# stateless-consensus/phant

Measured on AMD Instinct MI355X. Metric: mpt_proofs_verified_per_sec_depth8, higher is better.
Workload: dtype u64; 1 GPU; config3: 100000 synthetic depth-8 account proofs per GPU against one state root (7 x 532 B full branches + 112 B leaf, 3868 B and 29 Keccak-f per proof, 1% corrupted/exclusion, no cross-proof dedup); every launch sequence in flight verifies its own witness (seeds 2..3: distinct data per slot), 30 back-to-back passes per timed step; parallelism=key-sharded x1, verify_mode=flat, streams=2

## Files before the change

### phant_amd/csrc/mpt_verify_v3.hip

```cpp
#include <phant_platform.h>

#include "launch.h"
#include "mpt_verify_one.hip.h"
#include "coop_sponge.hip.h"
#include "verify_hash.hip.h"

namespace phant {
namespace v3 {
using namespace vh;

constexpr uint32_t HDR_PFN_BROKEN = 9;
constexpr uint32_t HDR_SLOW = 10;
constexpr uint32_t HDR_OPENED = 11;
constexpr uint32_t HDR_PARITY = 15;
constexpr uint32_t HDR_STAT = 1024;
constexpr uint32_t HDR_STAT_STRIPES = 16;
constexpr uint32_t HDR_STAT_WORDS = HDR_STAT_STRIPES * N_CLASS;
constexpr uint32_t HDR_STAT_END = HDR_STAT + 2u * HDR_STAT_WORDS;
constexpr uint32_t HDR_CUR = 256;
constexpr uint32_t HDR_WORDS = 768;
constexpr size_t HEADER_BYTES = 8192;
static_assert(HDR_STAT_END <= VERIFY_HEADER_WORDS && 4u * VERIFY_HEADER_WORDS <= HEADER_BYTES,
              "capi.hip copies VERIFY_HEADER_WORDS words back for the statistics");

PHANT_DEV uint32_t cursor_word(uint32_t cls, uint32_t stripe) { return HDR_CUR + 32u * stripe + cls; }



PHANT_DEV uint64_t key_prefix64(const uint8_t* __restrict__ key, uint32_t key_len) {
    uint64_t kb = 0;
    const uint32_t take = key_len < 8u ? key_len : 8u;
    for (uint32_t t = 0; t < take; ++t) kb |= (uint64_t)key[t] << (56u - 8u * t);
    return kb;
}
PHANT_DEV uint64_t key_prefix64_wide(const uint8_t* __restrict__ key, uint32_t key_len) {
    if (key_len < 8u) return key_prefix64(key, key_len);
    struct __attribute__((packed, aligned(1))) U64u { unsigned long long v; };
    return __builtin_bswap64(reinterpret_cast<const U64u*>(key)->v);
}
PHANT_DEV bool same_prefix(uint64_t x, uint64_t y, uint32_t d) { return d == 0u || ((x ^ y) >> (64u - 4u * d)) == 0ull; }
PHANT_DEV uint64_t group_hash(uint64_t kb, uint32_t root, uint32_t d) {
    const uint64_t pre = d ? (kb >> (64u - 4u * d)) : 0ull;
    uint64_t h = pre ^ ((uint64_t)(d + 1u) << 58) ^ ((uint64_t)root * 0x9E3779B97F4A7C15ull);
    h ^= h >> 33;
    h *= 0xff51afd7ed558ccdull;
    h ^= h >> 33;
    h *= 0xc4ceb9fe1a85ec53ull;
    h ^= h >> 33;
    return h;
}
PHANT_DEV uint32_t direct_index(uint64_t kb, uint32_t root, uint32_t d, uint32_t n_roots) {
    uint32_t width = 1u, below = 0u;
    for (uint32_t t = 0; t < d; ++t) {
        below += width;
        width <<= 4;
    }
    const uint32_t pre = d ? (uint32_t)(kb >> (64u - 4u * d)) : 0u;
    return n_roots * below + root * width + pre;
}
PHANT_DEV uint32_t slot_a(uint64_t h, uint32_t mask) { return (uint32_t)h & mask; }
PHANT_DEV uint32_t slot_b(uint64_t h, uint32_t mask) { return (uint32_t)(h >> 24) & mask; }

struct Args {
    VerifyArgs v;
    uint32_t total_nodes;
    uint32_t shallow;
    uint32_t direct;
    uint32_t* dtab;
    uint64_t* table;
    uint32_t tmask;
    uint32_t* rep;
    uint2* ent;
    uint32_t stripe_cap;
    uint32_t* hdr;
    uint32_t* digest;
    uint8_t* nstat;
};

PHANT_DEV void beside_the_hashing() { __builtin_amdgcn_s_setprio(3); }

__global__ void __launch_bounds__(256) zero_kernel(uint4* p, size_t n16, uint32_t* fail_count, uint32_t n_roots) {
    beside_the_hashing();
    const size_t i = (size_t)blockIdx.x * 256u + threadIdx.x;
    if (i < n16) p[i] = make_uint4(0u, 0u, 0u, 0u);
    if (fail_count)
        for (size_t r = i; r < n_roots; r += (size_t)gridDim.x * 256u) fail_count[r] = 0u;
}

struct ShallowLane {
    uint32_t p, d, j, root, len;
    uint64_t kb;
    bool act;
    bool valid;
    bool group;
    bool broken;
};
PHANT_DEV ShallowLane shallow_node(const Args& a, uint32_t p, uint32_t d) {
    ShallowLane L;
    L.p = p;
    L.d = d;
    L.j = 0;
    L.root = 0;
    L.len = 0;
    L.kb = 0;
    L.act = L.valid = L.group = L.broken = false;
    if (L.p >= a.v.n) return L;
    const uint32_t first = a.v.proof_first_node[L.p], last = a.v.proof_first_node[L.p + 1];
    if (last < first) {
        L.broken = L.d == 0u;
        return L;
    }
    if (last > a.total_nodes) return L;
    const uint32_t nn = 2u * a.v.key_len, cnt = last - first;
    const uint32_t end = cnt <= nn ? cnt : nn + 1u;
    if (L.d >= end) return L;
    L.act = true;
    L.j = first + L.d;
    L.root = a.v.root_idx ? a.v.root_idx[L.p] : 0u;
    const uint64_t e = a.v.node_off[L.j + 1], b = a.v.node_off[L.j];
    if (e >= b && e <= a.v.nodes_len && e - b <= 0x7fffffffull) {
        L.valid = true;
        L.len = (uint32_t)(e - b);
    }
    L.group = L.valid && L.len >= RATE && L.root < a.v.n_roots;
    if (L.group) L.kb = key_prefix64(a.v.keys + (uint64_t)a.v.key_len * L.p, a.v.key_len);
    return L;
}
PHANT_DEV ShallowLane shallow_lane(const Args& a, uint32_t g) {
    const uint32_t p = g / a.shallow;
    return shallow_node(a, p, g - p * a.shallow);
}

PHANT_DEV void clear_launch_state(const Args& a, uint32_t g, size_t lanes) {
    const uint32_t other = HDR_STAT + HDR_STAT_WORDS * ((a.hdr[HDR_PARITY] & 1u) ^ 1u);
    for (size_t i = g; i < HDR_WORDS + HDR_STAT_WORDS; i += lanes) {
        if (i < HDR_WORDS) {
            if (i != HDR_PARITY) a.hdr[i] = 0u;
        } else {
            a.hdr[other + (i - HDR_WORDS)] = 0u;
        }
    }
    if (a.v.fail_count)
        for (size_t r = g; r < a.v.n_roots; r += lanes) a.v.fail_count[r] = 0u;
}

__global__ void __launch_bounds__(256) propose_kernel(const Args a) {
    beside_the_hashing();
    const uint32_t g = blockIdx.x * 256u + threadIdx.x;
    clear_launch_state(a, g, (size_t)gridDim.x * 256u);
    const ShallowLane L = shallow_lane(a, g);
    if (L.act) a.nstat[L.j] = 0u;
    if (!L.group) return;
    if (L.d < a.direct) {
        a.dtab[direct_index(L.kb, L.root, L.d, a.v.n_roots)] = L.j + 1u;
    } else {
        const uint64_t h = group_hash(L.kb, L.root, L.d);
        const uint64_t entry = ((uint64_t)L.p << 32) | (uint64_t)(L.j + 1u);
        a.table[slot_a(h, a.tmask)] = entry;
        a.table[slot_b(h, a.tmask)] = entry;
    }
}

PHANT_DEV bool entry_matches(const Args& a, uint64_t en, const ShallowLane& L, uint32_t& node) {
    const uint32_t pr = (uint32_t)(en >> 32), j1 = (uint32_t)en;
    if (j1 == 0u || pr >= a.v.n) return false;
    node = j1 - 1u;
    if (pr == L.p) return node == L.j;
    const uint32_t f = a.v.proof_first_node[pr], l = a.v.proof_first_node[pr + 1];
    if (l < f || l > a.total_nodes || node < f || node >= l || node - f != L.d) return false;
    if ((a.v.root_idx ? a.v.root_idx[pr] : 0u) != L.root) return false;
    return same_prefix(key_prefix64(a.v.keys + (uint64_t)a.v.key_len * pr, a.v.key_len), L.kb, L.d);
}

PHANT_DEV uint64_t ent_index(const Args& a, uint32_t cls, uint32_t stripe, uint32_t at) {
    return ((uint64_t)cls * STRIPES + stripe) * a.stripe_cap + at;
}

PHANT_DEV bool wave_bytes_equal(const uint8_t* x, const uint8_t* y, uint32_t len, uint32_t lane) {
    uint32_t diff = 0;
    const uint32_t full = len & ~15u;
    for (uint32_t o = 16u * lane; o < full; o += 1024u) {
        const uint4 p = load16u(x + o), q = load16u(y + o);
        diff |= (p.x ^ q.x) | (p.y ^ q.y) | (p.z ^ q.z) | (p.w ^ q.w);
    }
    if (lane < (len & 15u)) diff |= (uint32_t)(x[full + lane] ^ y[full + lane]);
    return __ballot(diff != 0) == 0ull;
}

constexpr int COMPARE_UNROLL = 4;

__global__ void __launch_bounds__(256) PHANT_NUM_VGPR(48) dedup_kernel(const Args a) {
    constexpr uint32_t WAVES = 4;
    __shared__ uint32_t s_cnt[WAVES][N_LIST];
    __shared__ uint32_t s_base[N_LIST];
    beside_the_hashing();
    const uint32_t tid = threadIdx.x, lane = tid & 63u, wave = tid >> 6;
    const uint32_t NT = a.total_nodes;
    if (tid < WAVES * N_LIST) (&s_cnt[0][0])[tid] = 0u;
    const ShallowLane L = shallow_lane(a, blockIdx.x * 256u + tid);
    if (L.broken) a.hdr[HDR_PFN_BROKEN] = 1u;

    const uint32_t j = L.j;
    uint32_t cand = j;
    uint64_t b = 0, cb = 0;
    if (L.group) {
        uint32_t c = j;
        if (L.d < a.direct) {
            const uint32_t t = a.dtab[direct_index(L.kb, L.root, L.d, a.v.n_roots)];
            if (t) c = t - 1u;
        } else {
            const uint64_t h = group_hash(L.kb, L.root, L.d);
            uint32_t node;
            if (entry_matches(a, a.table[slot_a(h, a.tmask)], L, node)) c = node;
            else if (entry_matches(a, a.table[slot_b(h, a.tmask)], L, node)) c = node;
        }
        if (c != j && c < NT) {
            const uint64_t c0 = a.v.node_off[c], c1 = a.v.node_off[c + 1];
            if (c1 >= c0 && c1 <= a.v.nodes_len && c1 - c0 == L.len) {
                cand = c;
                cb = c0;
                b = a.v.node_off[j];
            }
        }
    }

    const uint32_t coff = 16u * (lane & 31u);
    const bool upper = lane >= 32u;
    const uint32_t b_lo = (uint32_t)b, b_hi = (uint32_t)(b >> 32), cb_lo = (uint32_t)cb, cb_hi = (uint32_t)(cb >> 32);
    bool differs = false;
    const bool is532 = cand != j && L.len == BRANCH_LEN;
    unsigned long long todo = __ballot(is532);
    while (todo) {
        uint32_t i0[COMPARE_UNROLL], i1[COMPARE_UNROLL];
        uint4 x[COMPARE_UNROLL], y[COMPARE_UNROLL];
        uint32_t i = 0;
#pragma unroll
        for (int u = 0; u < COMPARE_UNROLL; ++u) {
            if (todo) {
                i = (uint32_t)__builtin_ctzll(todo);
                todo &= todo - 1ull;
            }
            i0[u] = i;
            if (todo) {
                i = (uint32_t)__builtin_ctzll(todo);
                todo &= todo - 1ull;
            }
            i1[u] = i;
            const uint64_t own0 = lane_u64(b_lo, b_hi, i0[u]), own1 = lane_u64(b_lo, b_hi, i1[u]);
            const uint64_t oth0 = lane_u64(cb_lo, cb_hi, i0[u]), oth1 = lane_u64(cb_lo, cb_hi, i1[u]);
            x[u] = load16u(a.v.nodes + (upper ? own1 : own0) + coff);
            y[u] = load16u(a.v.nodes + (upper ? oth1 : oth0) + coff);
        }
#pragma unroll
        for (int u = 0; u < COMPARE_UNROLL; ++u) {
            uint32_t diff = x[u].x ^ y[u].x;
            diff = __builtin_amdgcn_bitop3_b32(x[u].y, y[u].y, diff, 0xBE);
            diff = __builtin_amdgcn_bitop3_b32(x[u].z, y[u].z, diff, 0xBE);
            diff = __builtin_amdgcn_bitop3_b32(x[u].w, y[u].w, diff, 0xBE);
            const unsigned long long m = __ballot(diff != 0);
            if ((uint32_t)m != 0u && lane == i0[u]) differs = true;
            if ((uint32_t)(m >> 32) != 0u && lane == i1[u]) differs = true;
        }
    }
    if (is532 && !differs) {
        const uint8_t* const own = a.v.nodes + b + (BRANCH_LEN - 28u);
        const uint8_t* const oth = a.v.nodes + cb + (BRANCH_LEN - 28u);
        const uint4 p0 = load16u(own), p1 = load16u(own + 12), q0 = load16u(oth), q1 = load16u(oth + 12);
        uint32_t diff = (p0.x ^ q0.x) | (p0.y ^ q0.y) | (p0.z ^ q0.z) | (p0.w ^ q0.w);
        diff |= (p1.x ^ q1.x) | (p1.y ^ q1.y) | (p1.z ^ q1.z) | (p1.w ^ q1.w);
        if (diff) differs = true;
    }
    todo = __ballot(cand != j && L.len != BRANCH_LEN);
    while (todo) {
        const uint32_t i = (uint32_t)__builtin_ctzll(todo);
        todo &= todo - 1ull;
        const uint32_t ll = lane_u32(L.len, i);
        const bool eq = wave_bytes_equal(a.v.nodes + lane_u64(b_lo, b_hi, i), a.v.nodes + lane_u64(cb_lo, cb_hi, i), ll, lane);
        if (lane == i && !eq) differs = true;
    }
    if (differs) cand = j;
    if (L.act) a.rep[j] = cand;

    const uint32_t cls = (L.act && L.valid && cand == j) ? node_list(L.len) : CLASS_NONE;
    uint32_t my_rank = 0;
    __syncthreads();
    todo = __ballot(cls != CLASS_NONE);
    while (todo) {
        const uint32_t c0 = lane_u32(cls, (uint32_t)__builtin_ctzll(todo));
        const unsigned long long m = __ballot(cls == c0);
        if (lane == 0) s_cnt[wave][c0] = (uint32_t)__popcll(m);
        if (cls == c0) my_rank = (uint32_t)__popcll(m & ((1ull << lane) - 1ull));
        todo &= ~m;
    }
    __syncthreads();
    const uint32_t stripe = blockIdx.x % STRIPES;
    if (tid < N_LIST) {
        uint32_t tot = 0;
        for (uint32_t w = 0; w < WAVES; ++w) tot += s_cnt[w][tid];
        s_base[tid] = tot ? atomicAdd(&a.hdr[cursor_word(tid, stripe)], tot) : 0u;
    }
    __syncthreads();
    if (cls != CLASS_NONE) {
        uint32_t at = s_base[cls] + my_rank;
        for (uint32_t w = 0; w < wave; ++w) at += s_cnt[w][cls];
        a.ent[ent_index(a, cls, stripe, at)] = make_uint2(j, L.p);
    }
}


PHANT_DEV const uint8_t* ref_location(const Args& a, uint32_t j, uint32_t d, uint32_t root, uint32_t nib_parent, uint64_t b) {
    if (d == 0u) return root < a.v.n_roots ? a.v.roots + 32ull * root : nullptr;
    if (nib_parent >= 16u) return nullptr;
    const uint64_t pb = a.v.node_off[j - 1u];
    if (pb > b || b - pb != BRANCH_LEN) return nullptr;
    return a.v.nodes + pb + (4u + 33u * nib_parent);
}

struct RefBytes { uint4 lo, hi; };
PHANT_DEV RefBytes load_ref(const uint8_t* q) {
    RefBytes r;
    r.lo = r.hi = make_uint4(0, 0, 0, 0);
    if (q) {
        r.lo = load16u(q);
        r.hi = load16u(q + 16);
    }
    return r;
}
PHANT_DEV bool digest_equals(const Sponge& s, const RefBytes& r) {
    const uint32_t diff = (s.lo[0] ^ r.lo.x) | (s.hi[0] ^ r.lo.y) | (s.lo[1] ^ r.lo.z) | (s.hi[1] ^ r.lo.w) |
                          (s.lo[2] ^ r.hi.x) | (s.hi[2] ^ r.hi.y) | (s.lo[3] ^ r.hi.z) | (s.hi[3] ^ r.hi.w);
    return diff == 0u;
}
PHANT_DEV void store_node_digest(const Args& a, uint32_t j, const Sponge& s) {
    uint4* o = reinterpret_cast<uint4*>(a.digest + 8ull * j);
    o[0] = make_uint4(s.lo[0], s.hi[0], s.lo[1], s.hi[1]);
    o[1] = make_uint4(s.lo[2], s.hi[2], s.lo[3], s.hi[3]);
}


PHANT_DEV bool list_role(const Args& a, uint32_t q, const uint32_t lane) {
    static_assert(N_QUEUE > 64u && N_QUEUE <= 128u, "two lists per lane");
    const uint32_t cnt_a = a.hdr[cursor_word(queue_class(lane), lane % STRIPES)];
    const uint32_t cnt_b = lane + 64u < N_QUEUE ? a.hdr[cursor_word(queue_class(lane + 64u), (lane + 64u) % STRIPES)] : 0u;
    const uint32_t ch_a = (cnt_a + 63u) / 64u, ch_b = (cnt_b + 63u) / 64u;
    const uint32_t incl_a = wave_inclusive_scan(ch_a, lane);
    uint32_t li, before, cnt;
    const unsigned long long m_a = __ballot(q < incl_a);
    if (m_a) {
        const uint32_t l = (uint32_t)__builtin_ctzll(m_a);
        li = l;
        before = lane_u32(incl_a, l) - lane_u32(ch_a, l);
        cnt = lane_u32(cnt_a, l);
    } else {
        const uint32_t incl_b = lane_u32(incl_a, 63u) + wave_inclusive_scan(ch_b, lane);
        const unsigned long long m_b = __ballot(q < incl_b);
        if (!m_b) return false;
        const uint32_t l = (uint32_t)__builtin_ctzll(m_b);
        li = l + 64u;
        before = lane_u32(incl_b, l) - lane_u32(ch_b, l);
        cnt = lane_u32(cnt_b, l);
    }
    const uint32_t cls = queue_class(li), stripe = li % STRIPES;
    uint32_t idx = (q - before) * 64u + lane;
    idx = idx < cnt ? idx : cnt - 1u;
    const uint2 en = a.ent[ent_index(a, cls, stripe, idx)];
    const uint32_t j = en.x;
    const uint8_t* const safe_end = a.v.nodes + a.v.nodes_len;
    const uint64_t b = a.v.node_off[j];
    const uint32_t len = (uint32_t)(a.v.node_off[j + 1] - b);
    const uint8_t* const p = a.v.nodes + b;

    const uint8_t* refp = nullptr;
    {
        const uint32_t owner = en.y;
        const uint32_t d = j - a.v.proof_first_node[owner];
        const uint32_t root = a.v.root_idx ? a.v.root_idx[owner] : 0u;
        uint32_t nibp = 16u;
        if (d >= 1u && d - 1u < 2u * a.v.key_len) nibp = key_nibble(a.v.keys + (uint64_t)a.v.key_len * owner, d - 1u);
        refp = ref_location(a, j, d, root, nibp, b);
    }
    const RefBytes ref = load_ref(refp);

    Sponge s;
    uint32_t bad;
    const uint32_t len0 = (uint32_t)__builtin_amdgcn_readfirstlane(len);
    if (cls == LIST_B532) {
        bad = hash_b532<true>(s, p);
    } else if (cls == 0u && __ballot(len != len0 || p + RATE > safe_end) == 0ull) {
        hash_short_uniform(s, p, len0);
        bad = 1u;
    } else {
        hash_any(s, p, len, safe_end);
        bad = 1u;
    }
    uint32_t ns = NS_HASHED | (bad == 0u ? NS_CANON : 0u);
    if (refp) ns |= NS_LINK_CHECKED | (digest_equals(s, ref) ? NS_LINK_OK : 0u);
    a.nstat[j] = (uint8_t)ns;
    store_node_digest(a, j, s);
    return true;
}

constexpr uint32_t DEEP_LEVELS = 8;

template <bool SOLO>
PHANT_DEV void deep_role(const Args& a, const uint32_t w, const uint32_t lane, const uint32_t waves_per_level, const uint32_t levels,
                         uint32_t (&s_ref)[8][256]) {
    const uint32_t level = w / waves_per_level;
    if (level >= levels) return;
    const uint32_t p = (w % waves_per_level) * 64u + lane;
    const uint8_t* const safe_end = a.v.nodes + a.v.nodes_len;
    const uint32_t nn = 2u * a.v.key_len;
    uint32_t hashed[N_CLASS] = {0, 0, 0, 0, 0, 0, 0, 0};
    const uint32_t stat_buf = a.hdr[HDR_PARITY] & 1u;
    for (uint32_t d = a.shallow + level;; d += levels) {
        uint32_t first = 0, count = 0, root = 0;
        if (p < a.v.n) {
            first = a.v.proof_first_node[p];
            const uint32_t last = a.v.proof_first_node[p + 1];
            if (last >= first && last <= a.total_nodes) count = last - first;
            if constexpr (SOLO) {
                if (last < first) a.hdr[HDR_PFN_BROKEN] = 1u;
            }
            if (a.v.root_idx) root = a.v.root_idx[p];
        }
        if (__ballot(d < count) == 0ull) break;
        const uint32_t j = first + d;
        bool active = d < count;
        uint64_t b = 0;
        uint32_t len = 0;
        if (active) {
            const uint64_t e = a.v.node_off[j + 1];
            b = a.v.node_off[j];
            active = e >= b && e <= a.v.nodes_len && e - b <= 0x7fffffffull;
            len = active ? (uint32_t)(e - b) : 0u;
            if (!active) a.nstat[j] = 0u;
        }
        const bool roomy = a.v.nodes_len >= BRANCH_LEN;
        const uint8_t* const ptr = a.v.nodes + (active ? b : 0ull);
        const uint8_t* refp = nullptr;
        if (active) {
            const uint8_t* const key = a.v.keys + (uint64_t)a.v.key_len * p;
            const uint32_t nibp = (d >= 1u && d - 1u < nn) ? key_nibble(key, d - 1u) : 16u;
            refp = ref_location(a, j, d, root, nibp, b);
        }
        {
            const RefBytes ref = load_ref(refp);
            const uint32_t t = threadIdx.x;
            s_ref[0][t] = ref.lo.x; s_ref[1][t] = ref.lo.y; s_ref[2][t] = ref.lo.z; s_ref[3][t] = ref.lo.w;
            s_ref[4][t] = ref.hi.x; s_ref[5][t] = ref.hi.y; s_ref[6][t] = ref.hi.z; s_ref[7][t] = ref.hi.w;
        }
        {
            const uint32_t cls = len / RATE < N_CLASS ? len / RATE : N_CLASS - 1u;
#pragma unroll
            for (uint32_t c = 0; c < N_CLASS; ++c) hashed[c] += (uint32_t)__popcll(__ballot(active && cls == c));
        }
        enum : uint32_t { F_ACTIVE = 1u, F_REF = 2u, F_CANON = 4u };
        uint32_t flags = (active ? F_ACTIVE : 0u) | (refp != nullptr ? F_REF : 0u);
        Sponge s;
        const bool is532 = active && len == BRANCH_LEN;
        if (roomy && __ballot(is532) != 0ull) {
            const uint32_t bad = hash_b532<true>(s, is532 ? ptr : a.v.nodes);
            if (is532 && bad == 0u) flags |= F_CANON;
        }
        const bool rest = active && !(roomy && is532);
        if (__ballot(rest) != 0ull) {
            const uint32_t len0 = (uint32_t)__builtin_amdgcn_readfirstlane(len);
            if (len0 < RATE && __ballot(!rest || len != len0 || ptr + RATE > safe_end) == 0ull) {
                hash_short_uniform(s, ptr, len0);
            } else if (rest) {
                hash_any(s, ptr, len, safe_end);
            }
        }
        if (flags & F_ACTIVE) {
            const uint32_t j = a.v.proof_first_node[p] + d;
            uint32_t ns = NS_HASHED | ((flags & F_CANON) ? NS_CANON : 0u);
            if (flags & F_REF) {
                const uint32_t t = threadIdx.x;
                RefBytes ref;
                ref.lo = make_uint4(s_ref[0][t], s_ref[1][t], s_ref[2][t], s_ref[3][t]);
                ref.hi = make_uint4(s_ref[4][t], s_ref[5][t], s_ref[6][t], s_ref[7][t]);
                ns |= NS_LINK_CHECKED | (digest_equals(s, ref) ? NS_LINK_OK : 0u);
            }
            a.nstat[j] = (uint8_t)ns;
            store_node_digest(a, j, s);
        }
    }
    if (lane < N_CLASS) {
        uint32_t mine = 0;
#pragma unroll
        for (uint32_t c = 0; c < N_CLASS; ++c) mine = lane == c ? hashed[c] : mine;
        if (mine) atomicAdd(&a.hdr[HDR_STAT + HDR_STAT_WORDS * stat_buf + N_CLASS * (w % HDR_STAT_STRIPES) + lane], mine);
    }
}

template <bool SOLO>
__global__ void __launch_bounds__(256, 4) hash_deep_kernel(const Args a, const uint32_t waves_per_level, const uint32_t levels) {
    __shared__ uint32_t s_ref[8][256];
    const uint32_t w = (uint32_t)__builtin_amdgcn_readfirstlane(blockIdx.x * 4u + (threadIdx.x >> 6));
    deep_role<SOLO>(a, w, threadIdx.x & 63u, waves_per_level, levels, s_ref);
}
constexpr uint32_t COOP_MAX_NODES = 2048;
constexpr uint32_t WAVE_MAX_NODES = 2048;
constexpr uint32_t NO_STAT = 0xffffffffu;
PHANT_DEV void coop_node(const Args& a, const CoopLane& c, const uint32_t l, const uint32_t base, const bool present, const uint32_t p,
                         const uint32_t j, const uint32_t d, const uint32_t root, const uint32_t stat_word) {
    struct __attribute__((packed, aligned(1))) U64 { unsigned long long v; };
    const uint32_t nn = 2u * a.v.key_len;
    bool active = false;
    uint32_t len = 0;
    uint64_t b = 0;
    if (present) {
        const uint64_t e = a.v.node_off[j + 1];
        b = a.v.node_off[j];
        active = e >= b && e <= a.v.nodes_len && e - b <= 0x7fffffffull;
        len = active ? (uint32_t)(e - b) : 0u;
        if (!active && l == 0) a.nstat[j] = 0u;
    }
    const uint8_t* const ptr = a.v.nodes + (active ? b : 0ull);
    const uint8_t* refp = nullptr;
    if (active) {
        const uint8_t* const key = a.v.keys + (uint64_t)a.v.key_len * p;
        refp = ref_location(a, j, d, root, (d >= 1u && d - 1u < nn) ? key_nibble(key, d - 1u) : 16u, b);
    }
    const uint32_t nb = active ? len / RATE + 1u : 0u;
    const uint32_t nb_other = __shfl(nb, (int)(base ^ 32u), 64);
    const uint32_t nb_max = nb > nb_other ? nb : nb_other;
    const bool branch = active && len == BRANCH_LEN;
    uint32_t lo = 0, hi = 0, dlo = 0, dhi = 0, bad = 0;
    for (uint32_t k = 0; k < nb_max; ++k) {
        if (k < nb && l < 17u) {
            const uint32_t off = k * RATE + 8u * l;
            unsigned long long w = 0;
            if (off + 8u <= len) {
                w = reinterpret_cast<const U64*>(ptr + off)->v;
            } else {
#pragma unroll
                for (uint32_t t = 0; t < 8u; ++t) {
                    const uint32_t q = off + t;
                    if (q < len) w |= (unsigned long long)ptr[q] << (8u * t);
                    else if (q == len) w |= 0x01ull << (8u * t);
                }
            }
            if (k + 1u == nb && l == 16u) w |= 0x80ull << 56;
            if (branch) {
#pragma unroll
                for (uint32_t t = 0; t < 8u; ++t) {
                    const uint32_t q = off + t;
                    const uint32_t byte = (uint32_t)(w >> (8u * t)) & 0xffu;
                    const int want = q == 0u ? 0xf9 : q == 1u ? 0x02 : q == 2u ? 0x11 : q == BRANCH_LEN - 1u ? 0x80 : (q < BRANCH_LEN && (q - 3u) % 33u == 0u) ? 0xa0 : -1;
                    if (want >= 0 && byte != (uint32_t)want) bad = 1u;
                }
            }
            lo ^= (uint32_t)w;
            hi ^= (uint32_t)(w >> 32);
        }
        coop_permute(c, lo, hi);
        if (k + 1u == nb) {
            dlo = lo;
            dhi = hi;
        }
    }
    bool ne = false;
    if (refp && l < 4u) {
        const unsigned long long r = reinterpret_cast<const U64*>(refp + 8u * l)->v;
        ne = (uint32_t)r != dlo || (uint32_t)(r >> 32) != dhi;
    }
    const uint32_t any_bad = (uint32_t)(__ballot(bad != 0u) >> base), any_ne = (uint32_t)(__ballot(ne) >> base);
    if (active) {
        uint32_t ns = NS_HASHED | ((branch && any_bad == 0u) ? NS_CANON : 0u);
        if (refp) ns |= NS_LINK_CHECKED | (any_ne == 0u ? NS_LINK_OK : 0u);
        if (l < 4u) {
            a.digest[8ull * j + 2u * l] = dlo;
            a.digest[8ull * j + 2u * l + 1u] = dhi;
        }
        if (l == 0) {
            a.nstat[j] = (uint8_t)ns;
            const uint32_t cls = len / RATE < N_CLASS ? len / RATE : N_CLASS - 1u;
            if (stat_word != NO_STAT) atomicAdd(&a.hdr[stat_word + cls], 1u);
        }
    }
}

__global__ void __launch_bounds__(256) hash_coop_kernel(const Args a, const uint32_t levels) {
    const uint32_t tid = threadIdx.x, l = tid & 31u, base = tid & 32u;
    const uint32_t h = blockIdx.x * (blockDim.x >> 5) + (tid >> 5);
    const uint32_t p = h / levels, level = h % levels;
    uint32_t first = 0, count = 0, root = 0;
    if (p < a.v.n) {
        first = a.v.proof_first_node[p];
        const uint32_t last = a.v.proof_first_node[p + 1];
        if (last >= first && last <= a.total_nodes) count = last - first;
        if (last < first && l == 0) a.hdr[HDR_PFN_BROKEN] = 1u;
        if (a.v.root_idx) root = a.v.root_idx[p];
    }
    const uint32_t stat_word = HDR_STAT + HDR_STAT_WORDS * (a.hdr[HDR_PARITY] & 1u) + N_CLASS * (h % HDR_STAT_STRIPES);
    const CoopLane c = coop_lane(l, base, gridDim.x * (blockDim.x >> 6) <= 1024u);
    for (uint32_t d = level;; d += levels) {
        if (__ballot(d < count) == 0ull) break;
        coop_node(a, c, l, base, d < count, p, first + d, d, root, stat_word);
    }
}

PHANT_DEV void wave_node(const Args& a, const WaveLane& c, const uint32_t l, const uint32_t p, const uint32_t j, const uint32_t d, const uint32_t root,
                         const uint32_t stat_word) {
    struct __attribute__((packed, aligned(1))) U64 { unsigned long long v; };
    const uint32_t nn = 2u * a.v.key_len;
    const uint64_t e = a.v.node_off[j + 1], b = a.v.node_off[j];
    const bool active = e >= b && e <= a.v.nodes_len && e - b <= 0x7fffffffull;
    if (!active) {
        if (l == 0) a.nstat[j] = 0u;
        return;
    }
    const uint32_t len = (uint32_t)(e - b);
    const uint8_t* const ptr = a.v.nodes + b;
    const uint8_t* const key = a.v.keys + (uint64_t)a.v.key_len * p;
    const uint8_t* const refp = ref_location(a, j, d, root, (d >= 1u && d - 1u < nn) ? key_nibble(key, d - 1u) : 16u, b);
    const uint32_t nb = len / RATE + 1u;
    const bool branch = len == BRANCH_LEN;
    uint32_t lo = 0, hi = 0, bad = 0;
    for (uint32_t k = 0; k < nb; ++k) {
        if (c.word < 17u) {
            const uint32_t off = k * RATE + 8u * c.word;
            unsigned long long w = 0;
            if (off + 8u <= len) {
                w = reinterpret_cast<const U64*>(ptr + off)->v;
            } else {
#pragma unroll
                for (uint32_t t = 0; t < 8u; ++t) {
                    const uint32_t q = off + t;
                    if (q < len) w |= (unsigned long long)ptr[q] << (8u * t);
                    else if (q == len) w |= 0x01ull << (8u * t);
                }
            }
            if (k + 1u == nb && c.word == 16u) w |= 0x80ull << 56;
            if (branch) {
#pragma unroll
                for (uint32_t t = 0; t < 8u; ++t) {
                    const uint32_t q = off + t;
                    const uint32_t byte = (uint32_t)(w >> (8u * t)) & 0xffu;
                    const int want = q == 0u ? 0xf9 : q == 1u ? 0x02 : q == 2u ? 0x11 : q == BRANCH_LEN - 1u ? 0x80 : (q < BRANCH_LEN && (q - 3u) % 33u == 0u) ? 0xa0 : -1;
                    if (want >= 0 && byte != (uint32_t)want) bad = 1u;
                }
            }
            lo ^= (uint32_t)w;
            hi ^= (uint32_t)(w >> 32);
        }
        wave_permute(c, lo, hi);
    }
    bool ne = false;
    if (refp && l < 4u) {
        const unsigned long long r = reinterpret_cast<const U64*>(refp + 8u * l)->v;
        ne = (uint32_t)r != lo || (uint32_t)(r >> 32) != hi;
    }
    const bool any_bad = __ballot(bad != 0u) != 0ull, any_ne = __ballot(ne) != 0ull;
    uint32_t ns = NS_HASHED | ((branch && !any_bad) ? NS_CANON : 0u);
    if (refp) ns |= NS_LINK_CHECKED | (!any_ne ? NS_LINK_OK : 0u);
    if (l < 4u) {
        a.digest[8ull * j + 2u * l] = lo;
        a.digest[8ull * j + 2u * l + 1u] = hi;
    }
    if (l == 0) {
        a.nstat[j] = (uint8_t)ns;
        const uint32_t cls = len / RATE < N_CLASS ? len / RATE : N_CLASS - 1u;
        if (stat_word != NO_STAT) atomicAdd(&a.hdr[stat_word + cls], 1u);
    }
}

__global__ void __launch_bounds__(256) hash_wave_kernel(const Args a, const uint32_t levels) {
    const uint32_t tid = threadIdx.x, l = tid & 63u;
    const uint32_t h = blockIdx.x * (blockDim.x >> 6) + (tid >> 6);
    const uint32_t p = h / levels, level = h % levels;
    if (p >= a.v.n) return;
    const uint32_t first = a.v.proof_first_node[p], last = a.v.proof_first_node[p + 1];
    uint32_t count = 0;
    if (last >= first && last <= a.total_nodes) count = last - first;
    if (last < first && l == 0) a.hdr[HDR_PFN_BROKEN] = 1u;
    const uint32_t root = a.v.root_idx ? a.v.root_idx[p] : 0u;
    const uint32_t stat_word = HDR_STAT + HDR_STAT_WORDS * (a.hdr[HDR_PARITY] & 1u) + N_CLASS * (h % HDR_STAT_STRIPES);
    const WaveLane c = wave_lane(l);
    for (uint32_t d = level; d < count; d += levels) wave_node(a, c, l, p, first + d, d, root, stat_word);
}

__global__ void __launch_bounds__(256, 4) hash_list_kernel(const Args a) {
    __builtin_amdgcn_s_setprio(2);
    const uint32_t q = (uint32_t)__builtin_amdgcn_readfirstlane(blockIdx.x * 4u + (threadIdx.x >> 6));
    (void)list_role(a, q, threadIdx.x & 63u);
}

enum : uint32_t { LINK_GENERIC = 0, LINK_FAST = 1, LINK_HASH_OK = 2, LINK_BAD_HASH = 3 };

PHANT_DEV uint32_t code_of(uint32_t ns, bool has_nibble) {
    if (!(ns & NS_HASHED) || !(ns & NS_LINK_CHECKED)) return LINK_GENERIC;
    if (!(ns & NS_LINK_OK)) return LINK_BAD_HASH;
    return (has_nibble && (ns & NS_CANON)) ? LINK_FAST : LINK_HASH_OK;
}


template <bool DIRECT>
__global__ void __launch_bounds__(256) walk_kernel(const Args a) {
    __shared__ uint32_t s_stage[256 * WALK_SLOT_DW];
    beside_the_hashing();
    const uint32_t i = blockIdx.x * 256u + threadIdx.x;
    const bool in = i < a.v.n;
    uint32_t status = PHANT_PROOF_PRESENT;
    uint32_t r = 0;
    if (in) {
        uint32_t* const slot = s_stage + threadIdx.x * WALK_SLOT_DW;
        const uint8_t* const slot_node = reinterpret_cast<const uint8_t*>(slot);
        const uint8_t* const nodes_end = a.v.nodes + a.v.nodes_len;
        uint64_t voff = 0;
        uint32_t vlen = 0;
        const uint32_t first = a.v.proof_first_node[i], last = a.v.proof_first_node[i + 1];
        r = a.v.root_idx ? a.v.root_idx[i] : 0u;
        if (last < first || last > a.total_nodes || r >= a.v.n_roots) {
            status = PHANT_PROOF_BAD_INPUT;
        } else if (last == first) {
            uint32_t rw[8];
            GlobalBytes rb{a.v.roots + 32ull * r};
#pragma unroll
            for (int k = 0; k < 8; ++k) rw[k] = rb.u32(4 * k);
            status = is_empty_root(rw) ? PHANT_PROOF_ABSENT : PHANT_PROOF_INVALID_EMPTY;
        } else if (a.hdr[HDR_PFN_BROKEN] != 0u) {
            status = STATUS_NEEDS_SLOW;
        } else {
            const uint8_t* const key = a.v.keys + (uint64_t)a.v.key_len * i;
            const uint32_t nn = 2u * a.v.key_len;
            uint32_t sx = 0;
            if constexpr (!DIRECT) {
                const uint32_t cnt = last - first, end = cnt <= nn ? cnt : nn + 1u;
                sx = end < a.shallow ? end : a.shallow;
            }
            const uint8_t* const slot_key = reinterpret_cast<const uint8_t*>(slot + WALK_STAGE_BYTES / 4);
            const bool key_in_lds = a.v.key_len <= WALK_KEY_BYTES;
            if (key_in_lds) {
                uint8_t* kdst = reinterpret_cast<uint8_t*>(slot + WALK_STAGE_BYTES / 4);
                for (uint32_t t = 0; t < a.v.key_len; ++t) kdst[t] = key[t];
            }
            WalkState w;
            w.pos = 0;
            w.status = PHANT_PROOF_BAD_INPUT;
            w.value_pay = w.value_len = w.ref_pay = w.ref_total = 0;
            uint32_t used = first;
            status = 0xffffffffu;

            bool hash_known = false;
            uint32_t rprev = 0;
            for (bool run = true; run && used < last;) {
                const uint32_t base = used, dbase = used - first;
                const uint8_t* lp = a.nstat + base;
                const uint32_t c0 = load4u(lp), c1 = load4u(lp + 4);
                uint32_t rj[8], nsr[8], rpar[8];
                if constexpr (!DIRECT) {
                    if (dbase < sx) {
                        const uint8_t* rp = reinterpret_cast<const uint8_t*>(a.rep + base);
                        const uint4 r0 = load16u(rp), r1 = load16u(rp + 16);
                        rj[0] = r0.x; rj[1] = r0.y; rj[2] = r0.z; rj[3] = r0.w;
                        rj[4] = r1.x; rj[5] = r1.y; rj[6] = r1.z; rj[7] = r1.w;
#pragma unroll
                        for (int u = 0; u < 8; ++u) {
                            const bool sh = dbase + u < sx && base + u < last && rj[u] < a.total_nodes;
                            rj[u] = sh ? rj[u] : base + u;
                        }
#pragma unroll
                        for (int u = 0; u < 8; ++u) {
                            const bool copy = rj[u] != base + u;
                            nsr[u] = copy ? a.nstat[rj[u]] : 0u;
                            rpar[u] = (copy && rj[u] >= 1u && dbase + u >= 1u) ? a.rep[rj[u] - 1u] : 0xffffffffu;
                        }
                    } else {
#pragma unroll
                        for (int u = 0; u < 8; ++u) {
                            rj[u] = base + u;
                            nsr[u] = 0u;
                            rpar[u] = 0xffffffffu;
                        }
                    }
                }
#pragma unroll
                for (int u = 0; u < 8; ++u) {
                    if (!run || used >= last) continue;
                    const uint32_t own = ((u < 4 ? c0 : c1) >> (8 * (u & 3))) & 0xffu;
                    uint32_t c, me = used;
                    if constexpr (DIRECT) {
                        c = code_of(own, w.pos < nn);
                    } else {
                        me = rj[u];
                        if (me == used) c = code_of(own, w.pos < nn);
                        else if (used == first || rpar[u] == rprev) c = code_of(nsr[u], w.pos < nn);
                        else if (!(nsr[u] & NS_HASHED)) c = LINK_GENERIC;
                        else {
                            const uint8_t* rb = a.v.nodes + a.v.node_off[used - 1u] + (4u + 33u * key_nibble(key, w.pos - 1u));
                            const uint4 w0 = load16u(rb), w1 = load16u(rb + 16);
                            const uint4* dg = reinterpret_cast<const uint4*>(a.digest + 8ull * me);
                            const uint4 d0 = dg[0], d1 = dg[1];
                            const uint32_t diff = (d0.x ^ w0.x) | (d0.y ^ w0.y) | (d0.z ^ w0.z) | (d0.w ^ w0.w) |
                                                  (d1.x ^ w1.x) | (d1.y ^ w1.y) | (d1.z ^ w1.z) | (d1.w ^ w1.w);
                            c = diff ? LINK_BAD_HASH : ((w.pos < nn && (nsr[u] & NS_CANON)) ? LINK_FAST : LINK_HASH_OK);
                        }
                    }
                    if (c == LINK_FAST) {
                        ++used;
                        w.pos += 1;
                        rprev = me;
                    } else {
                        run = false;
                        if (c == LINK_BAD_HASH) status = PHANT_PROOF_BAD_HASH;
                        else hash_known = c == LINK_HASH_OK;
                    }
                }
            }

            uint32_t want[8] = {0, 0, 0, 0, 0, 0, 0, 0};
            if (status == 0xffffffffu && !hash_known) {
                if (used == first) {
                    GlobalBytes rb{a.v.roots + 32ull * r};
#pragma unroll
                    for (int k = 0; k < 8; ++k) want[k] = rb.u32(4 * k);
                } else {
                    const uint32_t nibp = key_nibble(key, w.pos - 1u);
                    const uint8_t* rb = a.v.nodes + a.v.node_off[used - 1u] + (4u + 33u * nibp);
                    const uint4 r0 = load16u(rb), r1 = load16u(rb + 16);
                    want[0] = r0.x; want[1] = r0.y; want[2] = r0.z; want[3] = r0.w;
                    want[4] = r1.x; want[5] = r1.y; want[6] = r1.z; want[7] = r1.w;
                }
            }
            bool by_hash = true;
            const uint8_t* cur = nullptr;
            uint32_t cur_len = 0, opened = 0;
            const uint8_t* staged_from = nullptr;
            for (;;) {
                if (status != 0xffffffffu) break;
                ++opened;
                if (by_hash) {
                    if (used == last) {
                        status = PHANT_PROOF_MISSING_NODE;
                        break;
                    }
                    const uint32_t j = used;
                    const uint64_t b = a.v.node_off[j], e = a.v.node_off[j + 1];
                    if (e < b || e > a.v.nodes_len || e - b > 0x7fffffffull) {
                        status = PHANT_PROOF_BAD_INPUT;
                        break;
                    }
                    cur = a.v.nodes + b;
                    cur_len = (uint32_t)(e - b);
                    ++used;
                    if (hash_known) {
                        hash_known = false;
                    } else {
                        uint32_t rj = j;
                        if constexpr (!DIRECT) {
                            if (j - first < sx) rj = a.rep[j];
                        }
                        if (!(rj < a.total_nodes && (a.nstat[rj] & NS_HASHED))) {
                            status = STATUS_NEEDS_SLOW;
                            break;
                        }
                        const uint4* dg = reinterpret_cast<const uint4*>(a.digest + 8ull * rj);
                        const uint4 d0 = dg[0], d1 = dg[1];
                        const uint32_t diff = (d0.x ^ want[0]) | (d0.y ^ want[1]) | (d0.z ^ want[2]) | (d0.w ^ want[3]) |
                                              (d1.x ^ want[4]) | (d1.y ^ want[5]) | (d1.z ^ want[6]) | (d1.w ^ want[7]);
                        if (diff) {
                            status = PHANT_PROOF_BAD_HASH;
                            break;
                        }
                        if ((a.nstat[rj] & NS_CANON) && w.pos < nn) {
                            const uint8_t* rb = cur + (4u + 33u * key_nibble(key, w.pos));
                            const uint4 r0 = load16u(rb), r1 = load16u(rb + 16);
                            want[0] = r0.x; want[1] = r0.y; want[2] = r0.z; want[3] = r0.w;
                            want[4] = r1.x; want[5] = r1.y; want[6] = r1.z; want[7] = r1.w;
                            w.pos += 1;
                            continue;
                        }
                    }
                    staged_from = nullptr;
                    const uint32_t padded = (cur_len + 15u) & ~15u;
                    if (cur_len <= WALK_STAGE_BYTES && cur + padded <= nodes_end) {
                        for (uint32_t o = 0; o < padded; o += 16u) {
                            const uint4 q = load16u(cur + o);
                            slot[o / 4u] = q.x;
                            slot[o / 4u + 1u] = q.y;
                            slot[o / 4u + 2u] = q.z;
                            slot[o / 4u + 3u] = q.w;
                        }
                        staged_from = cur;
                    }
                }
                auto step_from = [&](const uint8_t* nb, const uint8_t* kp) __attribute__((always_inline)) -> uint32_t {
                    GlobalBytes nd{nb};
                    const uint32_t st = walk_node(nd, cur_len, kp, nn, w);
                    if (st == STEP_HASH) {
#pragma unroll
                        for (int k = 0; k < 8; ++k) want[k] = nd.u32(w.ref_pay + 4 * k);
                    }
                    return st;
                };
                uint32_t step;
                if (!key_in_lds) step = step_from(cur, key);
                else if (staged_from) step = step_from(slot_node + (cur - staged_from), slot_key);
                else step = step_from(cur, slot_key);
                if (step == STEP_DONE) break;
                if (step == STEP_HASH) {
                    by_hash = true;
                } else {
                    cur = cur + w.ref_pay;
                    cur_len = w.ref_total;
                    by_hash = false;
                }
            }
            if (opened > 1u) atomicAdd(&a.hdr[HDR_OPENED], opened);
            if (status == 0xffffffffu) {
                status = w.status;
                if (status == PHANT_PROOF_PRESENT || status == PHANT_PROOF_ABSENT) {
                    if (used != last) {
                        status = PHANT_PROOF_EXTRA_NODES;
                    } else if (status == PHANT_PROOF_PRESENT) {
                        voff = (uint64_t)(cur - a.v.nodes) + w.value_pay;
                        vlen = w.value_len;
                    }
                }
            }
        }
        if (status == STATUS_NEEDS_SLOW) {
            atomicAdd(&a.hdr[HDR_SLOW], 1u);
            status = verify_one(a.v, i, voff, vlen);
        }
        a.v.status[i] = (uint8_t)status;
        if (a.v.value_off) a.v.value_off[i] = voff;
        if (a.v.value_len) a.v.value_len[i] = vlen;
    }
    if (blockIdx.x == 0 && threadIdx.x == 0) a.hdr[HDR_PARITY] ^= 1u;
    if (a.v.fail_count) {
        const bool bad = in && !(status == PHANT_PROOF_PRESENT || status == PHANT_PROOF_ABSENT);
        if (a.v.root_idx == nullptr || a.v.n_roots == 1) {
            const unsigned long long m = __ballot(bad);
            if ((threadIdx.x & 63u) == 0 && m) atomicAdd(&a.v.fail_count[0], (uint32_t)__popcll(m));
        } else if (bad) {
            atomicAdd(&a.v.fail_count[r < a.v.n_roots ? r : 0u], 1u);
        }
    }
}

__global__ void __launch_bounds__(256) stream_read_kernel(const uint4* __restrict__ p, size_t n16, uint32_t* sink, size_t mask) {
    const size_t stride = (size_t)gridDim.x * 256u;
    size_t i = (size_t)blockIdx.x * 256u + threadIdx.x;
    uint4 acc = make_uint4(0u, 0u, 0u, 0u);
    for (; i + 7u * stride < n16; i += 8u * stride) {
        uint4 v[8];
#pragma unroll
        for (int u = 0; u < 8; ++u) v[u] = p[(i + (size_t)u * stride) & mask];
#pragma unroll
        for (int u = 0; u < 8; ++u) {
            acc.x ^= v[u].x;
            acc.y ^= v[u].y;
            acc.z ^= v[u].z;
            acc.w ^= v[u].w;
        }
    }
    for (; i < n16; i += stride) {
        const uint4 v = p[i & mask];
        acc.x ^= v.x;
        acc.y ^= v.y;
        acc.z ^= v.z;
        acc.w ^= v.w;
    }
    const uint32_t x = acc.x ^ acc.y ^ acc.z ^ acc.w;
    if (x == 0x9e3779b9u && sink) sink[blockIdx.x & 255u] = x;
}

static size_t rnd256(size_t x) { return (x + 255) / 256 * 256; }

constexpr uint64_t HASH_EVERYTHING_BELOW_BYTES = 72000000ull;

static uint32_t shallow_levels(uint32_t n, uint32_t n_roots, uint64_t nodes_len, int32_t forced) {
    if (forced >= 0) return (uint32_t)forced < MAX_SHALLOW ? (uint32_t)forced : MAX_SHALLOW;
    if (n < 2 || nodes_len < HASH_EVERYTHING_BELOW_BYTES) return 0;
    uint64_t n_eff = n;
    if (n_roots > 1u) {
        uint64_t r = 1;
        while ((r + 1) * (r + 1) <= n_roots) ++r;
        n_eff = n / r ? n / r : 1;
    }
    uint32_t s = 1;
    uint64_t groups = 16;
    while (s < MAX_SHALLOW && groups <= 4ull * n_eff) {
        ++s;
        groups *= 16;
    }
    return s;
}

constexpr uint64_t DIRECT_MAX_ENTRIES = 1ull << 21;
static uint32_t direct_levels(uint32_t n_roots, uint32_t shallow, uint64_t& entries) {
    uint32_t d = 0;
    uint64_t below = 0, width = 1;
    entries = 0;
    while (d < shallow && (below + width) * n_roots <= DIRECT_MAX_ENTRIES) {
        below += width;
        width *= 16;
        ++d;
        entries = below * n_roots;
    }
    return d;
}

static uint32_t table_entries(uint32_t n, uint32_t n_roots, uint32_t direct, uint32_t shallow, uint32_t total_nodes) {
    uint64_t per_root = 0, g = 1;
    for (uint32_t d = 0; d < shallow && per_root < (1ull << 40); ++d, g *= 16)
        if (d >= direct) per_root += g;
    uint64_t groups = per_root * (n_roots ? n_roots : 1u);
    const uint64_t by_nodes = (uint64_t)n * (shallow - direct) < total_nodes ? (uint64_t)n * (shallow - direct) : total_nodes;
    if (groups > by_nodes) groups = by_nodes;
    uint32_t t = 1024;
    while (t < 4 * groups && t < (1u << 26)) t <<= 1;
    return t;
}

struct Layout {
    size_t nstat, dtab, table, rep, ent, digest, end;
    uint32_t stripe_cap;
};
static Layout layout(uint32_t total_nodes, uint32_t te, uint64_t direct_entries, uint64_t lanes) {
    const size_t tn = total_nodes;
    Layout l;
    const uint64_t wgs = (lanes + 255u) / 256u;
    l.stripe_cap = (uint32_t)((wgs + STRIPES - 1u) / STRIPES * 256u);
    size_t p = HEADER_BYTES;
    l.nstat = p;  p += rnd256(tn + 16);
    l.dtab = p;   p += rnd256((size_t)direct_entries * 4);
    l.table = p;  p += rnd256((size_t)te * 8);
    l.rep = p;    p += rnd256(tn * 4 + 64);
    l.ent = p;    p += rnd256((size_t)N_LIST * STRIPES * l.stripe_cap * 8u);
    l.digest = p; p += rnd256(tn * 32);
    l.end = p + 1024;
    return l;
}

size_t workspace_bytes(uint32_t total_nodes) {
    uint32_t t = 1024;
    while (t < 4ull * total_nodes && t < (1u << 26)) t <<= 1;
    const uint64_t lanes = (uint64_t)total_nodes + 256u * STRIPES;
    return layout(total_nodes, t, DIRECT_MAX_ENTRIES, lanes).end;
}

static void bind(Args& a, uint8_t* ws, const Layout& l, uint32_t te) {
    a.hdr = reinterpret_cast<uint32_t*>(ws);
    a.nstat = ws + l.nstat;
    a.dtab = reinterpret_cast<uint32_t*>(ws + l.dtab);
    a.table = reinterpret_cast<uint64_t*>(ws + l.table);
    a.tmask = te - 1u;
    a.rep = reinterpret_cast<uint32_t*>(ws + l.rep);
    a.ent = reinterpret_cast<uint2*>(ws + l.ent);
    a.stripe_cap = l.stripe_cap;
    a.digest = reinterpret_cast<uint32_t*>(ws + l.digest);
}

}

size_t verify_workspace_bytes(uint32_t total_nodes) { return v3::workspace_bytes(total_nodes); }

hipError_t launch_mpt_verify(const VerifyArgs& v_in, uint32_t total_nodes, uint8_t* ws, int32_t dedup_levels,
                                hipStream_t st, const FlatSide* side, const VerifyTune& tune) {
    using namespace v3;
    VerifyArgs v = v_in;
    v.total_nodes = total_nodes;
    if (v.n == 0) return hipSuccess;
    Args a;
    a.v = v;
    a.total_nodes = total_nodes;
    a.shallow = shallow_levels(v.n, v.n_roots, v.nodes_len, dedup_levels);
    while (a.shallow && (uint64_t)v.n * a.shallow > (uint64_t)total_nodes + 256u * STRIPES) --a.shallow;
    if (tune.last_shallow) *tune.last_shallow = total_nodes ? a.shallow : 0u;
    uint64_t direct_entries = 0;
    a.direct = direct_levels(v.n_roots, a.shallow, direct_entries);
    const uint32_t te = table_entries(v.n, v.n_roots, a.direct, a.shallow, total_nodes);
    const uint64_t lanes = (uint64_t)v.n * a.shallow;
    const Layout l = layout(total_nodes, te, direct_entries, lanes);
    bind(a, ws, l, te);
    hipError_t e = hipSuccess;
    const uint32_t pg = (v.n + 255u) / 256u;
    const uint32_t wpl = (v.n + 63u) / 64u;
    const uint64_t avg_len = total_nodes ? (total_nodes + v.n - 1u) / v.n : 0u;
    const uint32_t deep_levels = avg_len + 1u <= a.shallow ? 1u
                                 : (uint32_t)(avg_len + 1u - a.shallow < DEEP_LEVELS ? avg_len + 1u - a.shallow : DEEP_LEVELS);
    const uint32_t deep_wgs = (wpl * deep_levels + 3u) / 4u;
    if (tune.last_form) *tune.last_form = (a.shallow == 0u || total_nodes == 0u) ? 0u : 1u;
    if (a.shallow == 0u || total_nodes == 0u) {
        a.shallow = 0;
        const size_t zero_n16 = l.dtab / 16;
        hipLaunchKernelGGL(zero_kernel, dim3((uint32_t)((zero_n16 + 255) / 256)), dim3(256), 0, st, reinterpret_cast<uint4*>(ws),
                           zero_n16, v.fail_count, v.n_roots);
        const uint64_t halves = (uint64_t)v.n * deep_levels;
        if (total_nodes && total_nodes <= tune.coop_max && !tune.no_coop && halves <= 4ull * COOP_MAX_NODES)
            if (halves <= WAVE_MAX_NODES && !tune.no_wave) {
                if (halves <= 512u) hipLaunchKernelGGL(hash_wave_kernel, dim3((uint32_t)halves), dim3(64), 0, st, a, deep_levels);
                else hipLaunchKernelGGL(hash_wave_kernel, dim3((uint32_t)((halves + 3u) / 4u)), dim3(256), 0, st, a, deep_levels);
            } else if (halves <= 1024u) {
                hipLaunchKernelGGL(hash_coop_kernel, dim3((uint32_t)((halves + 1u) / 2u)), dim3(64), 0, st, a, deep_levels);
            } else {
                hipLaunchKernelGGL(hash_coop_kernel, dim3((uint32_t)((halves + 7u) / 8u)), dim3(256), 0, st, a, deep_levels);
            }
        else if (total_nodes)
            hipLaunchKernelGGL(hash_deep_kernel<true>, dim3(deep_wgs), dim3(256), 0, st, a, wpl, deep_levels);
        hipLaunchKernelGGL(walk_kernel<true>, dim3(pg), dim3(256), 0, st, a);
        return hipGetLastError();
    }
    const uint32_t sg = (uint32_t)((lanes + 255u) / 256u);
    const bool two = side && side->stream && side->fork && side->join && !tune.serial;
    hipStream_t hs = two ? side->stream : st;
    const uint64_t listed = lanes < total_nodes ? lanes : total_nodes;
    const uint32_t list_wgs = (uint32_t)((listed + 255u) / 256u) + (N_QUEUE + 3u) / 4u;
    const uint32_t hash_lds = two ? tune.hash_lds : 0u;
    if (two) {
        if ((e = hipEventRecord(side->fork, st)) != hipSuccess) return e;
        if ((e = hipStreamWaitEvent(side->stream, side->fork, 0)) != hipSuccess) return e;
    }
    hipEvent_t* const kev = (!two && tune.serial) ? tune.kernel_ev : nullptr;
    auto mark = [&](int i) {
        if (kev && e == hipSuccess) e = hipEventRecord(kev[i], st);
    };
    if (tune.diag) {
        const bool three = two && side->stream2 && side->join2;
        hipStream_t h2 = three ? side->stream2 : st;
        if (two) {
            if ((e = hipEventRecord(side->fork, st)) != hipSuccess) return e;
            if ((e = hipStreamWaitEvent(side->stream, side->fork, 0)) != hipSuccess) return e;
            if (three && (e = hipStreamWaitEvent(side->stream2, side->fork, 0)) != hipSuccess) return e;
        }
        if (tune.diag & 1u) {
            const uint32_t lds = tune.diag == 3u ? hash_lds : 0u;
            hipLaunchKernelGGL(hash_deep_kernel<false>, dim3(deep_wgs), dim3(256), lds, hs, a, wpl, deep_levels);
            hipLaunchKernelGGL(hash_list_kernel, dim3(list_wgs), dim3(256), lds ? lds + 8192u : 0u, st, a);
        }
        if (tune.diag & 2u) {
            const uint32_t wgs = tune.diag_stream_wgs ? tune.diag_stream_wgs : 2048u;
            size_t mask = ~(size_t)0;
            if (tune.diag_stream_mb) {
                size_t r16 = (size_t)tune.diag_stream_mb << 16;
                while (r16 > v.nodes_len / 16u) r16 >>= 1;
                mask = r16 ? r16 - 1u : 0u;
            }
            hipLaunchKernelGGL(stream_read_kernel, dim3(wgs), dim3(256), 0, h2, reinterpret_cast<const uint4*>(v.nodes),
                               (size_t)(v.nodes_len / 16u), tune.diag_sink, mask);
        }
        if (two) {
            if ((e = hipEventRecord(side->join, side->stream)) != hipSuccess) return e;
            if ((e = hipStreamWaitEvent(st, side->join, 0)) != hipSuccess) return e;
            if (three) {
                if ((e = hipEventRecord(side->join2, side->stream2)) != hipSuccess) return e;
                if ((e = hipStreamWaitEvent(st, side->join2, 0)) != hipSuccess) return e;
            }
        }
        return hipGetLastError();
    }
    mark(0);
    hipLaunchKernelGGL(propose_kernel, dim3(sg), dim3(256), 0, st, a);
    mark(1);
    hipLaunchKernelGGL(hash_deep_kernel<false>, dim3(deep_wgs), dim3(256), hash_lds, hs, a, wpl, deep_levels);
    mark(2);
    if (two && (e = hipEventRecord(side->join, side->stream)) != hipSuccess) return e;
    hipLaunchKernelGGL(dedup_kernel, dim3(sg), dim3(256), 0, st, a);
    mark(3);
    hipLaunchKernelGGL(hash_list_kernel, dim3(list_wgs), dim3(256), hash_lds ? hash_lds + 8192u : 0u, st, a);
    mark(4);
    if (two && (e = hipStreamWaitEvent(st, side->join, 0)) != hipSuccess) return e;
    hipLaunchKernelGGL(walk_kernel<false>, dim3(pg), dim3(256), 0, st, a);
    mark(5);
    if (e != hipSuccess) return e;
    return hipGetLastError();
}

void verify_stats_from_header(const uint32_t* hdr, uint32_t hashed[8]) {
    using namespace v3;
    uint32_t lists[N_LIST];
    for (uint32_t c = 0; c < N_LIST; ++c) {
        lists[c] = 0;
        for (uint32_t s = 0; s < STRIPES; ++s) lists[c] += hdr[HDR_CUR + 32u * s + c];
    }
    const uint32_t buf = (hdr[HDR_PARITY] & 1u) ^ 1u;
    for (uint32_t c = 0; c < N_CLASS; ++c) {
        hashed[c] = lists[c];
        for (uint32_t s = 0; s < HDR_STAT_STRIPES; ++s) hashed[c] += hdr[HDR_STAT + HDR_STAT_WORDS * buf + N_CLASS * s + c];
    }
    hashed[BRANCH_LEN / RATE] += lists[LIST_B532];
}
void verify_tier_stats_from_header(const uint32_t* hdr, uint32_t out[4]) {
    using namespace v3;
    out[0] = out[1] = out[2] = out[3] = 0;
    for (uint32_t c = 0; c < N_LIST; ++c) {
        uint32_t cnt = 0;
        for (uint32_t s = 0; s < STRIPES; ++s) cnt += hdr[HDR_CUR + 32u * s + c];
        out[0] += cnt;
        out[1] += cnt * (c == LIST_B532 ? BRANCH_LEN / RATE + 1u : c + 1u);
    }
    const uint32_t buf = (hdr[HDR_PARITY] & 1u) ^ 1u;
    for (uint32_t c = 0; c < N_CLASS; ++c)
        for (uint32_t s = 0; s < HDR_STAT_STRIPES; ++s) {
            const uint32_t cnt = hdr[HDR_STAT + HDR_STAT_WORDS * buf + N_CLASS * s + c];
            out[2] += cnt;
            out[3] += cnt * (c + 1u);
        }
}
void verify_paths_from_header(const uint32_t* hdr, uint32_t out[2]) {
    out[0] = hdr[v3::HDR_SLOW];
    out[1] = hdr[v3::HDR_OPENED];
}

}
```

Measured before the change: 542.8 million proofs/s.

## Pack node offset, length and reference location into 16-byte queue descriptors

```diff
diff --git a/phant_amd/csrc/mpt_verify_v3.hip b/phant_amd/csrc/mpt_verify_v3.hip
--- a/phant_amd/csrc/mpt_verify_v3.hip
+++ b/phant_amd/csrc/mpt_verify_v3.hip
@@ -70,7 +70,7 @@
     uint64_t* table;
     uint32_t tmask;
     uint32_t* rep;
-    uint2* ent;
+    uint4* ent;
     uint32_t stripe_cap;
     uint32_t* hdr;
     uint32_t* digest;
@@ -89,6 +89,7 @@
 
 struct ShallowLane {
     uint32_t p, d, j, root, len;
+    uint64_t b;
     uint64_t kb;
     bool act;
     bool valid;
@@ -102,6 +103,7 @@
     L.j = 0;
     L.root = 0;
     L.len = 0;
+    L.b = 0;
     L.kb = 0;
     L.act = L.valid = L.group = L.broken = false;
     if (L.p >= a.v.n) return L;
@@ -121,6 +123,7 @@
     if (e >= b && e <= a.v.nodes_len && e - b <= 0x7fffffffull) {
         L.valid = true;
         L.len = (uint32_t)(e - b);
+        L.b = b;
     }
     L.group = L.valid && L.len >= RATE && L.root < a.v.n_roots;
     if (L.group) L.kb = key_prefix64(a.v.keys + (uint64_t)a.v.key_len * L.p, a.v.key_len);
@@ -161,6 +164,33 @@
     }
 }
 
+constexpr uint32_t DESC_LEN_BIG = 0x7fffffu;
+constexpr uint32_t DESC_ROOT = 0x80000000u;
+constexpr uint32_t DESC_NO_REF = 0xffffffffu;
+constexpr uint64_t DESC_MAX_OFF = 1ull << 40;
+
+PHANT_DEV uint4 node_desc(const Args& a, uint32_t j, uint32_t d, uint32_t root, uint32_t nibp, uint64_t b, uint32_t len) {
+    uint32_t w = DESC_NO_REF, flag = 0u;
+    if (d == 0u) {
+        if (root < a.v.n_roots) {
+            w = root;
+            flag = DESC_ROOT;
+        }
+    } else if (nibp < 16u) {
+        const uint64_t pb = a.v.node_off[j - 1u];
+        if (pb <= b && b - pb == BRANCH_LEN) w = nibp;
+    }
+    const bool fits = b < DESC_MAX_OFF && len < DESC_LEN_BIG;
+    const uint32_t y = fits ? (uint32_t)(b >> 32) | (len << 8) : DESC_LEN_BIG << 8;
+    return make_uint4(fits ? (uint32_t)b : 0u, y | flag, j, w);
+}
+PHANT_DEV uint32_t desc_len(const uint4& q) { return (q.y >> 8) & 0x7fffffu; }
+PHANT_DEV uint64_t desc_off(const uint4& q) { return ((uint64_t)(q.y & 0xffu) << 32) | (uint64_t)q.x; }
+PHANT_DEV const uint8_t* desc_ref(const Args& a, const uint4& q, uint64_t b) {
+    if (q.y & DESC_ROOT) return a.v.roots + 32ull * q.w;
+    return q.w < 16u ? a.v.nodes + (b - BRANCH_LEN + 4u + 33u * q.w) : nullptr;
+}
+
 PHANT_DEV bool entry_matches(const Args& a, uint64_t en, const ShallowLane& L, uint32_t& node) {
     const uint32_t pr = (uint32_t)(en >> 32), j1 = (uint32_t)en;
     if (j1 == 0u || pr >= a.v.n) return false;
@@ -202,7 +232,8 @@
 
     const uint32_t j = L.j;
     uint32_t cand = j;
-    uint64_t b = 0, cb = 0;
+    const uint64_t b = L.b;
+    uint64_t cb = 0;
     if (L.group) {
         uint32_t c = j;
         if (L.d < a.direct) {
@@ -219,7 +250,6 @@
             if (c1 >= c0 && c1 <= a.v.nodes_len && c1 - c0 == L.len) {
                 cand = c;
                 cb = c0;
-                b = a.v.node_off[j];
             }
         }
     }
@@ -282,6 +312,12 @@
     if (L.act) a.rep[j] = cand;
 
     const uint32_t cls = (L.act && L.valid && cand == j) ? node_list(L.len) : CLASS_NONE;
+    uint4 desc = make_uint4(0u, 0u, 0u, 0u);
+    if (cls != CLASS_NONE) {
+        const uint32_t nibp =
+            (L.d >= 1u && L.d - 1u < 2u * a.v.key_len) ? key_nibble(a.v.keys + (uint64_t)a.v.key_len * L.p, L.d - 1u) : 16u;
+        desc = node_desc(a, j, L.d, L.root, nibp, L.b, L.len);
+    }
     uint32_t my_rank = 0;
     __syncthreads();
     todo = __ballot(cls != CLASS_NONE);
@@ -303,7 +339,7 @@
     if (cls != CLASS_NONE) {
         uint32_t at = s_base[cls] + my_rank;
         for (uint32_t w = 0; w < wave; ++w) at += s_cnt[w][cls];
-        a.ent[ent_index(a, cls, stripe, at)] = make_uint2(j, L.p);
+        a.ent[ent_index(a, cls, stripe, at)] = desc;
     }
 }
 
@@ -363,22 +399,18 @@
     const uint32_t cls = queue_class(li), stripe = li % STRIPES;
     uint32_t idx = (q - before) * 64u + lane;
     idx = idx < cnt ? idx : cnt - 1u;
-    const uint2 en = a.ent[ent_index(a, cls, stripe, idx)];
-    const uint32_t j = en.x;
+    const uint4 en = a.ent[ent_index(a, cls, stripe, idx)];
+    const uint32_t j = en.z;
     const uint8_t* const safe_end = a.v.nodes + a.v.nodes_len;
-    const uint64_t b = a.v.node_off[j];
-    const uint32_t len = (uint32_t)(a.v.node_off[j + 1] - b);
+    uint64_t b = desc_off(en);
+    uint32_t len = desc_len(en);
+    if (len == DESC_LEN_BIG) {
+        b = a.v.node_off[j];
+        len = (uint32_t)(a.v.node_off[j + 1] - b);
+    }
     const uint8_t* const p = a.v.nodes + b;
 
-    const uint8_t* refp = nullptr;
-    {
-        const uint32_t owner = en.y;
-        const uint32_t d = j - a.v.proof_first_node[owner];
-        const uint32_t root = a.v.root_idx ? a.v.root_idx[owner] : 0u;
-        uint32_t nibp = 16u;
-        if (d >= 1u && d - 1u < 2u * a.v.key_len) nibp = key_nibble(a.v.keys + (uint64_t)a.v.key_len * owner, d - 1u);
-        refp = ref_location(a, j, d, root, nibp, b);
-    }
+    const uint8_t* const refp = desc_ref(a, en, b);
     const RefBytes ref = load_ref(refp);
 
     Sponge s;
@@ -1030,7 +1062,7 @@
     l.dtab = p;   p += rnd256((size_t)direct_entries * 4);
     l.table = p;  p += rnd256((size_t)te * 8);
     l.rep = p;    p += rnd256(tn * 4 + 64);
-    l.ent = p;    p += rnd256((size_t)N_LIST * STRIPES * l.stripe_cap * 8u);
+    l.ent = p;    p += rnd256((size_t)N_LIST * STRIPES * l.stripe_cap * 16u);
     l.digest = p; p += rnd256(tn * 32);
     l.end = p + 1024;
     return l;
@@ -1050,7 +1082,7 @@
     a.table = reinterpret_cast<uint64_t*>(ws + l.table);
     a.tmask = te - 1u;
     a.rep = reinterpret_cast<uint32_t*>(ws + l.rep);
-    a.ent = reinterpret_cast<uint2*>(ws + l.ent);
+    a.ent = reinterpret_cast<uint4*>(ws + l.ent);
     a.stripe_cap = l.stripe_cap;
     a.digest = reinterpret_cast<uint32_t*>(ws + l.digest);
 }
```

Result: no change. 539.4 million proofs/s, median of 2 (-0.6%).
